# JinPLu/VeloxSeg

Measured on AMD Instinct MI355X. Metric: training patches/s on 128^3 2-mod volumes (fwd+loss+bwd+allreduce+AdamW), higher is better.
Workload: dtype f32

## Files before the change

veloxseg_amd/csrc/pwa_fused.hip:

```cpp
#include "vx_common.h"
#include "../../include/veloxseg_hip.h"

typedef float vx_f32x4 __attribute__((ext_vector_type(4)));
#define VX_MFMA(a, b, c) __builtin_amdgcn_mfma_f32_16x16x4f32((a), (b), (c), 0, 0, 0)

namespace {
template <int T> struct Geo { static constexpr int NT = 16 * T; static constexpr int S = (T == 1) ? 20 : 64; };

template <int T, int NW, bool TR, class Epi>
__device__ __forceinline__ void tile_gemm(int nseg, const float* const (&w)[3], const int (&Kseg)[3], int wsm, int wsk, int Mrows, const float* __restrict__ in, Epi&& epi) {
    constexpr int S = Geo<T>::S;
    const int lane = threadIdx.x & 63, wave = threadIdx.x >> 6, r = lane & 15, q = lane >> 4;
    for (int mt = wave; mt * 16 < Mrows; mt += NW) {
        vx_f32x4 acc[T];
#pragma unroll
        for (int j = 0; j < T; ++j) acc[j] = (vx_f32x4){0.f, 0.f, 0.f, 0.f};
        int kin = 0;
        float a[4][4], an[4][4];
        typedef const __attribute__((address_space(1))) float* gcf;
        typedef const __attribute__((address_space(1))) vx_f32x4* gcf4;
        auto load_a = [&](float (&dst)[4][4], const float* __restrict__ wrow_, int K, int k0) {
            gcf wrow = (gcf)(unsigned long long)wrow_;
#pragma unroll
            for (int c = 0; c < 4; ++c) {
                const int kb = min(k0 + 16 * c, K - 16) + 4 * q;
                if (!TR) {
                    const vx_f32x4 t = *(gcf4)(wrow + kb);
                    dst[c][0] = t[0]; dst[c][1] = t[1]; dst[c][2] = t[2]; dst[c][3] = t[3];
                } else {
#pragma unroll
                    for (int i = 0; i < 4; ++i) dst[c][i] = wrow[(long)(kb + i) * wsk];
                }
            }
// ... 15 lines not shown
                                acc[0] = VX_MFMA(a[c][i], bv.x, acc[0]);
                                acc[1] = VX_MFMA(a[c][i], bv.y, acc[1]);
                                acc[2] = VX_MFMA(a[c][i], bv.z, acc[2]);
                                acc[3] = VX_MFMA(a[c][i], bv.w, acc[3]);
                            } else {
                                acc[0] = VX_MFMA(a[c][i], brow[i * S + r], acc[0]);
                            }
                        }
                    }
                }
                if (k0 + 64 < K) {
#pragma unroll
                    for (int c = 0; c < 4; ++c)
#pragma unroll
                        for (int i = 0; i < 4; ++i) a[c][i] = an[c][i];
                }
            }
            kin += K;
        }
        epi(mt, acc);
    }
}
template <int T, int NW, bool TR, class Epi>
__device__ __forceinline__ void tile_gemm1(const float* w, int K, int wsm, int wsk, int Mrows, const float* __restrict__ in, Epi&& epi) {
    const float* const ws[3] = {w, nullptr, nullptr};
    const int ks[3] = {K, 0, 0};
    tile_gemm<T, NW, TR>(1, ws, ks, wsm, wsk, Mrows, in, epi);
}

template <int T, int NW>
__device__ __forceinline__ void load_tile(float* __restrict__ dst, const float* __restrict__ src , int R, long V, long v0) {
    constexpr int S = Geo<T>::S, RP = 4 * NW, U = 8;
    const int cg = threadIdx.x & 15;
    for (int row0 = threadIdx.x >> 4; row0 < R; row0 += U * RP) {
        if constexpr (T == 4) {
            const long v = v0 + 4 * cg;
            const bool ok = v < V;
            const long vc = ok ? v : 0;
            float4 t[U];
#pragma unroll
            for (int u = 0; u < U; ++u) { const int row = min(row0 + u * RP, R - 1); t[u] = *reinterpret_cast<const float4*>(src + (long)row * V + vc); }
#pragma unroll
            for (int u = 0; u < U; ++u) {
                const int row = row0 + u * RP;
                if (row < R) *reinterpret_cast<float4*>(dst + row * S + 4 * cg) = ok ? t[u] : make_float4(0.f, 0.f, 0.f, 0.f);
            }
        } else {
            const long v = v0 + cg;
            const bool ok = v < V;
            const long vc = ok ? v : 0;
            float t[U];
#pragma unroll
            for (int u = 0; u < U; ++u) { const int row = min(row0 + u * RP, R - 1); t[u] = src[(long)row * V + vc]; }
#pragma unroll
            for (int u = 0; u < U; ++u) {
                const int row = row0 + u * RP;
                if (row < R) dst[row * S + cg] = ok ? t[u] : 0.0f;
            }
        }
    }
}

template <int T, int NW>
__device__ __forceinline__ void tile_ln_stats(const float* __restrict__ X, int C, float eps, float* __restrict__ red, float& mean, float& rstd) {
    constexpr int NT = Geo<T>::NT, S = Geo<T>::S, NP = 64 * NW / NT;
    const int col = threadIdx.x % NT, part = threadIdx.x / NT;
    float s = 0.0f;
    for (int c = part; c < C; c += NP) s += X[c * S + col];
    red[part * NT + col] = s;
    __syncthreads();
    float tot = 0.0f;
#pragma unroll 4
    for (int p_ = 0; p_ < NP; ++p_) tot += red[p_ * NT + col];
    mean = tot / (float)C;
    __syncthreads();
    float qq = 0.0f;
    for (int c = part; c < C; c += NP) { const float d = X[c * S + col] - mean; qq = fmaf(d, d, qq); }
    red[part * NT + col] = qq;
    __syncthreads();
    float var = 0.0f;
#pragma unroll 4
    for (int p_ = 0; p_ < NP; ++p_) var += red[p_ * NT + col];
    rstd = 1.0f / sqrtf(var / (float)C + eps);
}

__device__ __forceinline__ VxDropCtx drop_ctx_dev(const void* seed_ptr, unsigned long long site, float p) {
    VxDrop d;
    d.seed_ptr = p > 0.0f ? (const uint64_t*)seed_ptr : nullptr;
    d.stream = site;
    d.p = p;
    return vx_drop_ctx(d);
}
template <int T>
__device__ __forceinline__ void acc_masks(const VxDropCtx& dc, uint64_t row, long V, long v, float (&m)[4]) {
    if (!dc.on) { m[0] = m[1] = m[2] = m[3] = 1.0f; return; }
    if constexpr (T == 4) vx_masks_vox4(dc, row, V, v, m);
    else { m[0] = vx_drop1(dc, row * (uint64_t)V + (uint64_t)v); m[1] = m[2] = m[3] = 1.0f; }
}
}

struct VxLnPwMod {
    const float *x, *gamma, *beta;
// ... 33 lines not shown
        for (int u = 0; u < U; ++u) {
            const bool in = row0 + u * RP < C;
            const int so = (sub >> 2) * HW2 + ((sub >> 1) & 1) * (2 * gw) + (sub & 1);
            t[u] = xv[(long)c * cstride + so];
            if (in && row0 + (u + 1) * RP < C) {
                c += RP;
                while (c >= C0) { c -= C0; ++sub; }
            }
        }
#pragma unroll
        for (int u = 0; u < U; ++u) {
            const int rw = row0 + u * RP;
            if (rw < C) dst[rw * S + cg] = ok ? t[u] : 0.0f;
        }
    }
}

template <int NW>
__device__ __forceinline__ void stage_vec(float* __restrict__ dst, const float* __restrict__ src, int n, float fill) {
    for (int i = threadIdx.x; i < n; i += 64 * NW) dst[i] = src ? src[i] : fill;
}

template <int T, int NW>
__global__ void __launch_bounds__(64 * NW) vx_ln_pw_fwd_k(VxLnPw p) {
    constexpr int NT = Geo<T>::NT, S = Geo<T>::S, NP = 64 * NW / NT;
    extern __shared__ __attribute__((aligned(16))) float vx_pf_lds[];
    const VxLnPwMod& M = p.m[blockIdx.y];
    const int C = p.C;
    const int Jt = p.J[0] + p.J[1] + p.J[2];
    float* __restrict__ X = vx_pf_lds;
    float* __restrict__ red = X + C * S;
    float* __restrict__ gam = red + NP * NT;
    float* __restrict__ bet = gam + C;
    float* __restrict__ bia = bet + C;
    const int b = blockIdx.x / p.tiles_per_b;
    const long V = p.V, v0 = (long)(blockIdx.x % p.tiles_per_b) * NT;
    stage_vec<NW>(gam, M.gamma, C, 1.0f);
    stage_vec<NW>(bet, M.beta, C, 0.0f);
    {
        int j0 = 0;
        for (int sg = 0; sg < p.NS; ++sg) { stage_vec<NW>(bia + j0, M.b[sg], p.J[sg], 0.0f); j0 += p.J[sg]; }
    }
    if constexpr (T == 1) {
        if (p.s2d) load_tile_s2d<T, NW>(X, M.x + (long)b * C * V, C, p.C0, p.gh, p.gw, V, v0);
        else load_tile<T, NW>(X, M.x + (long)b * C * V, C, V, v0);
    } else load_tile<T, NW>(X, M.x + (long)b * C * V, C, V, v0);
    __syncthreads();
    float mean, rstd;
    tile_ln_stats<T, NW>(X, C, p.eps, red, mean, rstd);
    {
        const int col = threadIdx.x % NT, part = threadIdx.x / NT;
        const bool live = v0 + col < V;
        float* __restrict__ xn = M.xn ? M.xn + (long)b * C * V + v0 + col : nullptr;
        for (int c = part; c < C; c += NP) {
            const float n = fmaf(gam[c], (X[c * S + col] - mean) * rstd, bet[c]);
            X[c * S + col] = n;
            if (xn && live) xn[(long)c * V] = n;
        }
    }
    __syncthreads();
    const int lane = threadIdx.x & 63, r = lane & 15, q = lane >> 4;
    int j0 = 0;
    for (int sg = 0; sg < p.NS; ++sg) {
        const int J = p.J[sg];
        const float* __restrict__ bias = bia + j0;
        float* __restrict__ out = M.out[sg] + (long)b * J * V;
        tile_gemm1<T, NW, false>(M.w[sg], C, C, 1, J, X, [&](int mt, vx_f32x4 (&acc)[T]) {
#pragma unroll
            for (int reg = 0; reg < 4; ++reg) {
                const int m = 16 * mt + 4 * q + reg;
                const float bb = bias[m];
                if constexpr (T == 4) {
                    const long v = v0 + 4 * r;
                    if (v < V) *reinterpret_cast<float4*>(out + (long)m * V + v) = make_float4(acc[0][reg] + bb, acc[1][reg] + bb, acc[2][reg] + bb, acc[3][reg] + bb);
                } else {
                    const long v = v0 + r;
                    if (v < V) out[(long)m * V + v] = acc[0][reg] + bb;
                }
            }
        });
        j0 += J;
    }
}

struct VxLnPwBwdMod {
    const float *x, *gamma;
    const float* w[3];
    const float* dout[3];
    const float* dres;
    float* dx;
    float* part;
};
struct VxLnPwBwd {
    VxLnPwBwdMod m[4];
    int C, NS;
    int J[3];
    long V;
    int tiles_per_b;
    float eps;
    int s2d, C0, gh, gw;
};

template <int T, int NW>
__global__ void __launch_bounds__(64 * NW) vx_ln_pw_bwd_k(VxLnPwBwd p) {
    constexpr int NT = Geo<T>::NT, S = Geo<T>::S, NP = 64 * NW / NT;
    extern __shared__ __attribute__((aligned(16))) float vx_pf_lds[];
    const VxLnPwBwdMod& M = p.m[blockIdx.y];
    const int C = p.C;
    int Jt = 0;
    for (int sg = 0; sg < p.NS; ++sg) Jt += p.J[sg];
    float* __restrict__ D = vx_pf_lds;
    float* __restrict__ X = D + Jt * S;
    float* __restrict__ G = X + C * S;
    float* __restrict__ red = G + C * S;
    float* __restrict__ gam = red + 2 * NP * NT;
    const int b = blockIdx.x / p.tiles_per_b;
    const long V = p.V, v0 = (long)(blockIdx.x % p.tiles_per_b) * NT;
    stage_vec<NW>(gam, M.gamma, C, 1.0f);
    {
        int j0 = 0;
        for (int sg = 0; sg < p.NS; ++sg) {
            load_tile<T, NW>(D + j0 * S, M.dout[sg] + (long)b * p.J[sg] * V, p.J[sg], V, v0);
            j0 += p.J[sg];
        }
    }
    if constexpr (T == 1) {
        if (p.s2d) load_tile_s2d<T, NW>(X, M.x + (long)b * C * V, C, p.C0, p.gh, p.gw, V, v0);
        else load_tile<T, NW>(X, M.x + (long)b * C * V, C, V, v0);
    } else load_tile<T, NW>(X, M.x + (long)b * C * V, C, V, v0);
    __syncthreads();
    const int lane = threadIdx.x & 63, r = lane & 15, q = lane >> 4;
    {
        const float* const ws[3] = {M.w[0], M.w[1], M.w[2]};
        const int ks[3] = {p.J[0], p.J[1], p.J[2]};
        tile_gemm<T, NW, true>(p.NS, ws, ks, 1, C, C, D, [&](int mt, vx_f32x4 (&acc)[T]) {
#pragma unroll
            for (int reg = 0; reg < 4; ++reg) {
                const int m = 16 * mt + 4 * q + reg;
                if constexpr (T == 4) *reinterpret_cast<float4*>(G + m * S + 4 * r) = make_float4(acc[0][reg], acc[1][reg], acc[2][reg], acc[3][reg]);
                else G[m * S + r] = acc[0][reg];
            }
        });
    }
    float mean, rstd;
    tile_ln_stats<T, NW>(X, C, p.eps, red, mean, rstd);
    const bool has_res = M.dres != nullptr && Jt >= C;
    if (has_res) load_tile<T, NW>(D, M.dres + (long)b * C * V, C, V, v0);
    const int col = threadIdx.x % NT, part = threadIdx.x / NT;
    float s1 = 0.0f, s2 = 0.0f;
    for (int c = part; c < C; c += NP) {
        const float xh = (X[c * S + col] - mean) * rstd;
        const float g = G[c * S + col] * gam[c];
        s1 += g;
        s2 = fmaf(g, xh, s2);
    }
    __syncthreads();
    red[part * NT + col] = s1;
    red[(NP + part) * NT + col] = s2;
    __syncthreads();
    float t1 = 0.0f, t2 = 0.0f;
#pragma unroll 4
    for (int p_ = 0; p_ < NP; ++p_) { t1 += red[p_ * NT + col]; t2 += red[(NP + p_) * NT + col]; }
    t1 /= (float)C; t2 /= (float)C;
    const bool live = v0 + col < V;
    float* __restrict__ pp = M.part ? M.part + (long)blockIdx.x * 2 * C : nullptr;
    long s2d_base = 0, HW2 = 0, gd2 = 0;
    if (p.s2d) {
        const long v = live ? v0 + col : 0;
        const int w_ = (int)(v % p.gw), h_ = (int)((v / p.gw) % p.gh), d_ = (int)(v / ((long)p.gw * p.gh));
        HW2 = (long)(2 * p.gh) * (2 * p.gw);
        gd2 = 2 * (V / ((long)p.gh * p.gw));
        s2d_base = (long)b * C * V + (long)(2 * d_) * HW2 + (long)(2 * h_) * (2 * p.gw) + 2 * w_;
    }
    int ssub = p.s2d ? part / p.C0 : 0, sc0 = p.s2d ? part - ssub * p.C0 : 0;
    const long cstr2 = gd2 * HW2;
    for (int c = part; c < C; c += NP) {
        const float xh = (X[c * S + col] - mean) * rstd;
        const float dn = G[c * S + col];
        const float g = dn * gam[c];
        float dg = dn * xh, db = dn;
#pragma unroll
        for (int o = 1; o < NT; o <<= 1) { dg += __shfl_xor(dg, o, 64); db += __shfl_xor(db, o, 64); }
// ... 43 lines not shown
template <int T, int NW>
__global__ void __launch_bounds__(64 * NW) vx_pwa_post_fwd_k(VxPost p) {
    constexpr int NT = Geo<T>::NT, S = Geo<T>::S, NP = 64 * NW / NT;
    extern __shared__ __attribute__((aligned(16))) float vx_pf_lds[];
    const VxPostMod& M = p.m[blockIdx.y];
    const int C = p.C, Cv = p.Cv, R = p.R;
    float* __restrict__ Sx = vx_pf_lds;
    float* __restrict__ Y = Sx + Cv * S;
    float* __restrict__ N = Y + C * S;
    float* __restrict__ Hh = N + C * S;
    float* __restrict__ red = Hh + R * S;
    float* __restrict__ prm = red + NP * NT;
    float* __restrict__ bm = prm, *gam = prm + C, *bet = prm + 2 * C, *b2 = prm + 3 * C, *b1 = prm + 4 * C;
    const int b = blockIdx.x / p.tiles_per_b;
    const long V = p.V, v0 = (long)(blockIdx.x % p.tiles_per_b) * NT;
    const VxDropCtx dm = drop_ctx_dev(p.seed_ptr, M.site_mix, p.p_mix);
    const VxDropCtx d1 = drop_ctx_dev(p.seed_ptr, M.site1, p.p_ffn);
    const VxDropCtx d2 = drop_ctx_dev(p.seed_ptr, M.site2, p.p_ffn);
    stage_vec<NW>(bm, M.bm, C, 0.0f);
    stage_vec<NW>(gam, M.gamma, C, 1.0f);
    stage_vec<NW>(bet, M.beta, C, 0.0f);
    stage_vec<NW>(b2, M.b2, C, 0.0f);
    stage_vec<NW>(b1, M.b1, R, 0.0f);
    load_tile<T, NW>(Sx, M.s + (long)b * Cv * V, Cv, V, v0);
    load_tile<T, NW>(Y, M.x + (long)b * C * V, C, V, v0);
    __syncthreads();
    const int lane = threadIdx.x & 63, r = lane & 15, q = lane >> 4;
    const int cr = T * r;
    const long v = v0 + cr;
    const bool vlive = v < V;
    tile_gemm1<T, NW, false>(M.wm, Cv, Cv, 1, C, Sx, [&](int mt, vx_f32x4 (&acc)[T]) {
#pragma unroll
        for (int reg = 0; reg < 4; ++reg) {
            const int m = 16 * mt + 4 * q + reg;
            const long row = (long)b * C + m;
            float yv[T], mk[4];
            ldv<T>(Y + m * S + cr, yv);
            if (vlive) {
                acc_masks<T>(dm, (uint64_t)row, V, v, mk);
#pragma unroll
                for (int j = 0; j < T; ++j) yv[j] = fmaf(p.alpha, yv[j], (acc[j][reg] + bm[m]) * mk[j]);
                stv<T>(M.y + row * V + v, yv);
            } else {
#pragma unroll
                for (int j = 0; j < T; ++j) yv[j] = 0.0f;
            }
            stv<T>(Y + m * S + cr, yv);
        }
    });
    __syncthreads();
    float mean, rstd;
    tile_ln_stats<T, NW>(Y, C, p.eps, red, mean, rstd);
    {
        const int col = threadIdx.x % NT, part = threadIdx.x / NT;
        for (int c = part; c < C; c += NP) N[c * S + col] = fmaf(gam[c], (Y[c * S + col] - mean) * rstd, bet[c]);
    }
    __syncthreads();
    tile_gemm1<T, NW, false>(M.w1, C, C, 1, R, N, [&](int mt, vx_f32x4 (&acc)[T]) {
#pragma unroll
        for (int reg = 0; reg < 4; ++reg) {
            const int j = 16 * mt + 4 * q + reg;
            float hv[T], mk[4];
            if (vlive) {
                acc_masks<T>(d1, (uint64_t)((long)b * R + j), V, v, mk);
#pragma unroll
                for (int i = 0; i < T; ++i) hv[i] = vx_gelu_fast(acc[i][reg] + b1[j]) * mk[i];
            } else {
#pragma unroll
                for (int i = 0; i < T; ++i) hv[i] = 0.0f;
            }
            stv<T>(Hh + j * S + cr, hv);
        }
    });
    __syncthreads();
    tile_gemm1<T, NW, false>(M.w2, R, R, 1, C, Hh, [&](int mt, vx_f32x4 (&acc)[T]) {
#pragma unroll
        for (int reg = 0; reg < 4; ++reg) {
            const int m = 16 * mt + 4 * q + reg;
            if (vlive) {
                const long row = (long)b * C + m;
                float ov[T], mk[4];
                ldv<T>(Y + m * S + cr, ov);
                acc_masks<T>(d2, (uint64_t)row, V, v, mk);
#pragma unroll
                for (int i = 0; i < T; ++i) ov[i] = fmaf(acc[i][reg] + b2[m], mk[i], ov[i]);
                stv<T>(M.out + row * V + v, ov);
            }
        }
    });
}

template <int T, int NW>
__global__ void __launch_bounds__(64 * NW) vx_pwa_post_bwd_k(VxPost p) {
    constexpr int NT = Geo<T>::NT, S = Geo<T>::S, NP = 64 * NW / NT, NRP = 4 * NW;
    extern __shared__ __attribute__((aligned(16))) float vx_pf_lds[];
    const VxPostMod& M = p.m[blockIdx.y];
    const int C = p.C, Cv = p.Cv, R = p.R;
    float* __restrict__ DO = vx_pf_lds;
// ... 29 lines not shown
#pragma unroll
            for (int j = 0; j < T; ++j) g[j] *= mk[j];
            stv<T>(M.sc_dz + row * V + vq, g);
        } else {
#pragma unroll
            for (int j = 0; j < T; ++j) g[j] = 0.0f;
        }
        stv<T>(DZ + c * S + cq, g);
    }
    float mean, rstd;
    tile_ln_stats<T, NW>(Y, C, p.eps, red, mean, rstd);
    for (int c = part; c < C; c += NP) {
        const float xh = (Y[c * S + col] - mean) * rstd;
        const float n = fmaf(gam[c], xh, bet[c]);
        N[c * S + col] = n;
        Y[c * S + col] = xh;
        if (clive) M.sc_n[((long)b * C + c) * V + v0 + col] = n;
    }
    __syncthreads();
    const int lane = threadIdx.x & 63, r = lane & 15, q = lane >> 4;
    const int cr = T * r;
    const long v = v0 + cr;
    const bool vlive = v < V;
    tile_gemm1<T, NW, false>(M.w1, C, C, 1, R, N, [&](int mt, vx_f32x4 (&acc)[T]) {
#pragma unroll
        for (int reg = 0; reg < 4; ++reg) {
            const int j = 16 * mt + 4 * q + reg;
            float a[T];
#pragma unroll
            for (int i = 0; i < T; ++i) a[i] = acc[i][reg] + b1[j];
            stv<T>(A + j * S + cr, a);
            if (vlive) {
                const long row = (long)b * R + j;
                float mk[4];
                acc_masks<T>(d1, (uint64_t)row, V, v, mk);
#pragma unroll
                for (int i = 0; i < T; ++i) a[i] = vx_gelu_fast(a[i]) * mk[i];
                stv<T>(M.sc_h + row * V + v, a);
            }
        }
    });
    __syncthreads();
    tile_gemm1<T, NW, true>(M.w2, C, 1, R, R, DZ, [&](int mt, vx_f32x4 (&acc)[T]) {
#pragma unroll
        for (int reg = 0; reg < 4; ++reg) {
            const int j = 16 * mt + 4 * q + reg;
            const long row = (long)b * R + j;
            float da[T];
            if (vlive) {
                float mk[4];
                ldv<T>(A + j * S + cr, da);
                acc_masks<T>(d1, (uint64_t)row, V, v, mk);
#pragma unroll
                for (int i = 0; i < T; ++i) da[i] = acc[i][reg] * mk[i] * vx_gelu_grad_fast(da[i]);
                stv<T>(M.sc_da + row * V + v, da);
            } else {
#pragma unroll
                for (int i = 0; i < T; ++i) da[i] = 0.0f;
            }
            stv<T>(A + j * S + cr, da);
        }
    });
    __syncthreads();
    tile_gemm1<T, NW, true>(M.w1, R, 1, C, C, A, [&](int mt, vx_f32x4 (&acc)[T]) {
#pragma unroll
        for (int reg = 0; reg < 4; ++reg) {
            float dn[T];
#pragma unroll
            for (int i = 0; i < T; ++i) dn[i] = acc[i][reg];
            stv<T>(DZ + (16 * mt + 4 * q + reg) * S + cr, dn);
        }
    });
    __syncthreads();
    float s1 = 0.0f, s2 = 0.0f;
    for (int c = part; c < C; c += NP) {
        const float g = DZ[c * S + col] * gam[c];
        s1 += g;
        s2 = fmaf(g, Y[c * S + col], s2);
    }
    red[part * NT + col] = s1;
    red[(NP + part) * NT + col] = s2;
    __syncthreads();
    float t1 = 0.0f, t2 = 0.0f;
#pragma unroll 4
    for (int p_ = 0; p_ < NP; ++p_) { t1 += red[p_ * NT + col]; t2 += red[(NP + p_) * NT + col]; }
    t1 /= (float)C; t2 /= (float)C;
    float rs_[T], t1_[T], t2_[T];
// ... 13 lines not shown
        for (int j = 0; j < T; ++j) { dg = fmaf(dn[j], xh[j], dg); db += dn[j]; }
#pragma unroll
        for (int o = 1; o < 16; o <<= 1) { dg += __shfl_xor(dg, o, 64); db += __shfl_xor(db, o, 64); }
        if (qd == 0) { pp[c] = dg; pp[C + c] = db; }
        if (qlive) {
            float mk[4], dx[T];
            ldv<T>(DO + c * S + cq, dy);
            acc_masks<T>(dm, (uint64_t)row, V, vq, mk);
#pragma unroll
            for (int j = 0; j < T; ++j) {
                dy[j] += rs_[j] * (dn[j] * gam[c] - t1_[j] - xh[j] * t2_[j]);
                dx[j] = p.alpha * dy[j];
                dy[j] *= mk[j];
            }
            stv<T>(M.dxres + row * V + vq, dx);
            stv<T>(M.sc_dmix + row * V + vq, dy);
        } else {
#pragma unroll
            for (int j = 0; j < T; ++j) dy[j] = 0.0f;
        }
        stv<T>(N + c * S + cq, dy);
    }
    __syncthreads();
    tile_gemm1<T, NW, true>(M.wm, C, 1, Cv, Cv, N, [&](int mt, vx_f32x4 (&acc)[T]) {
#pragma unroll
        for (int reg = 0; reg < 4; ++reg) {
            const int m = 16 * mt + 4 * q + reg;
            if (vlive) {
                float o[T];
#pragma unroll
                for (int i = 0; i < T; ++i) o[i] = acc[i][reg];
                stv<T>(M.ds + ((long)b * Cv + m) * V + v, o);
            }
        }
    });
}

static inline int pf_tile_t(long V) { return ((V & 3) == 0 && V >= 2048) ? 4 : 1; }
static inline int pf_nw(long blocks) { return blocks < 256 ? 8 : 4; }

extern "C" int vx_ln_pw_tiles(int B, long V) {
    const int T = pf_tile_t(V);
    return B * vx_cdiv(V, 16 * T);
}

static size_t pf_lds_limit() {
    static size_t lim = 0;
// ... 155 lines not shown
}

struct VxInMlp {
    const float *o, *w1, *b1, *w2, *b2, *dout;
    const double* part;
    float* stats;
    float *out, *dn, *part_dn;
    float *sc_n, *sc_h, *sc_da, *sc_dz;
    int C, R, nparts, tiles_per_b;
    long V;
    float eps, p;
    unsigned long long site;
    const void* seed_ptr;
};
namespace {
template <int NW>
__device__ __forceinline__ void inmlp_stats(const VxInMlp& p, int b, float* __restrict__ mu, float* __restrict__ rs, bool writer) {
    for (int c = threadIdx.x; c < p.C; c += 64 * NW) {
        const long bc = (long)b * p.C + c;
        float mean, rstd;
        if (p.part != nullptr) {
            double s = 0.0, q = 0.0;
            const double* pp = p.part + bc * p.nparts * 2;
            for (int i = 0; i < p.nparts; ++i) { s += pp[2 * i]; q += pp[2 * i + 1]; }
            const double m = s / (double)p.V;
            double var = q / (double)p.V - m * m;
            var = var < 0.0 ? 0.0 : var;
            mean = (float)m;
            rstd = (float)(1.0 / sqrt(var + (double)p.eps));
            if (writer) { p.stats[2 * bc] = mean; p.stats[2 * bc + 1] = rstd; }
        } else {
            mean = p.stats[2 * bc];
            rstd = p.stats[2 * bc + 1];
        }
        mu[c] = mean;
        rs[c] = rstd;
    }
}
}

template <int NW>
__global__ void __launch_bounds__(64 * NW) vx_inmlp_fwd_k(VxInMlp p) {
    constexpr int T = 1, NT = 16, S = Geo<1>::S, NP = 64 * NW / NT;
    extern __shared__ __attribute__((aligned(16))) float vx_pf_lds[];
    const int C = p.C, R = p.R;
    float* __restrict__ O = vx_pf_lds;
    float* __restrict__ N = O + C * S;
    float* __restrict__ Hh = N + C * S;
    float* __restrict__ mu = Hh + R * S, *rs = mu + C, *b2 = rs + C, *b1 = b2 + C;
    const int b = blockIdx.x / p.tiles_per_b, tile = blockIdx.x % p.tiles_per_b;
    const long V = p.V, v0 = (long)tile * NT;
    const VxDropCtx d2 = drop_ctx_dev(p.seed_ptr, p.site, p.p);
    inmlp_stats<NW>(p, b, mu, rs, tile == 0);
    stage_vec<NW>(b2, p.b2, C, 0.0f);
    stage_vec<NW>(b1, p.b1, R, 0.0f);
    load_tile<T, NW>(O, p.o + (long)b * C * V, C, V, v0);
    __syncthreads();
    {
        const int col = threadIdx.x % NT, part = threadIdx.x / NT;
        for (int c = part; c < C; c += NP) N[c * S + col] = (O[c * S + col] - mu[c]) * rs[c];
    }
    __syncthreads();
    const int lane = threadIdx.x & 63, r = lane & 15, q = lane >> 4;
    const long v = v0 + r;
    const bool vlive = v < V;
    tile_gemm1<T, NW, false>(p.w1, C, C, 1, R, N, [&](int mt, vx_f32x4 (&acc)[T]) {
#pragma unroll
        for (int reg = 0; reg < 4; ++reg) {
            const int j = 16 * mt + 4 * q + reg;
            Hh[j * S + r] = vlive ? vx_gelu_fast(acc[0][reg] + b1[j]) : 0.0f;
        }
    });
    __syncthreads();
    tile_gemm1<T, NW, false>(p.w2, R, R, 1, C, Hh, [&](int mt, vx_f32x4 (&acc)[T]) {
#pragma unroll
        for (int reg = 0; reg < 4; ++reg) {
            const int m = 16 * mt + 4 * q + reg;
            if (vlive) {
                const long idx = ((long)b * C + m) * V + v;
                p.out[idx] = fmaf(acc[0][reg] + b2[m], vx_drop1(d2, (uint64_t)idx), O[m * S + r]);
            }
        }
    });
}

template <int NW>
__global__ void __launch_bounds__(64 * NW) vx_inmlp_bwd_k(VxInMlp p) {
    constexpr int T = 1, NT = 16, S = Geo<1>::S, NP = 64 * NW / NT;
    extern __shared__ __attribute__((aligned(16))) float vx_pf_lds[];
    const int C = p.C, R = p.R;
    float* __restrict__ DZ = vx_pf_lds;
    float* __restrict__ N = DZ + C * S;
    float* __restrict__ A = N + C * S;
    float* __restrict__ mu = A + R * S, *rs = mu + C, *b1 = rs + C;
    const int b = blockIdx.x / p.tiles_per_b, tile = blockIdx.x % p.tiles_per_b;
    const long V = p.V, v0 = (long)tile * NT;
    const VxDropCtx d2 = drop_ctx_dev(p.seed_ptr, p.site, p.p);
    const int col = threadIdx.x % NT, part = threadIdx.x / NT;
    const bool clive = v0 + col < V;
    inmlp_stats<NW>(p, b, mu, rs, false);
    stage_vec<NW>(b1, p.b1, R, 0.0f);
    load_tile<T, NW>(N, p.o + (long)b * C * V, C, V, v0);
    load_tile<T, NW>(DZ, p.dout + (long)b * C * V, C, V, v0);
    __syncthreads();
    for (int c = part; c < C; c += NP) {
        const long idx = ((long)b * C + c) * V + v0 + col;
        const float g = clive ? DZ[c * S + col] * vx_drop1(d2, (uint64_t)idx) : 0.0f;
        const float nh = clive ? (N[c * S + col] - mu[c]) * rs[c] : 0.0f;
        DZ[c * S + col] = g;
        N[c * S + col] = nh;
        if (clive) { p.sc_dz[idx] = g; p.sc_n[idx] = nh; }
    }
    __syncthreads();
    const int lane = threadIdx.x & 63, r = lane & 15, q = lane >> 4;
    const long v = v0 + r;
    const bool vlive = v < V;
    tile_gemm1<T, NW, false>(p.w1, C, C, 1, R, N, [&](int mt, vx_f32x4 (&acc)[T]) {
#pragma unroll
        for (int reg = 0; reg < 4; ++reg) {
            const int j = 16 * mt + 4 * q + reg;
            const float a = acc[0][reg] + b1[j];
            A[j * S + r] = a;
            if (vlive) p.sc_h[((long)b * R + j) * V + v] = vx_gelu_fast(a);
        }
    });
    __syncthreads();
    tile_gemm1<T, NW, true>(p.w2, C, 1, R, R, DZ, [&](int mt, vx_f32x4 (&acc)[T]) {
#pragma unroll
        for (int reg = 0; reg < 4; ++reg) {
            const int j = 16 * mt + 4 * q + reg;
            const float da = vlive ? acc[0][reg] * vx_gelu_grad_fast(A[j * S + r]) : 0.0f;
            A[j * S + r] = da;
            if (vlive) p.sc_da[((long)b * R + j) * V + v] = da;
        }
    });
    __syncthreads();
    tile_gemm1<T, NW, true>(p.w1, R, 1, C, C, A, [&](int mt, vx_f32x4 (&acc)[T]) {
#pragma unroll
        for (int reg = 0; reg < 4; ++reg) {
            const int m = 16 * mt + 4 * q + reg;
            const float dn = vlive ? acc[0][reg] : 0.0f;
            if (vlive) p.dn[((long)b * C + m) * V + v] = dn;
            float s1 = dn, s2 = dn * N[m * S + r];
#pragma unroll
            for (int o_ = 1; o_ < 16; o_ <<= 1) { s1 += __shfl_xor(s1, o_, 64); s2 += __shfl_xor(s2, o_, 64); }
            if (r == 0) {
                float* __restrict__ pp = p.part_dn + (((long)b * C + m) * p.tiles_per_b + tile) * 2;
                pp[0] = s1; pp[1] = s2;
            }
        }
    });
}

extern "C" int vx_inmlp_ok(int C, int R, long V) {
    if (C % 16 || R % 16 || C < 16 || R < 16 || C > 256 || V < 1) return 0;
    const size_t lds = ((size_t)(2 * C + R) * 20 + 3 * C + R) * sizeof(float);
    return lds <= pf_lds_budget() ? 1 : 0;
}
extern "C" int vx_inmlp_tiles(long V) { return vx_cdiv(V, 16); }

// ... 34 lines not shown
```

Baseline: 1118.

## Pipeline weight-fragment prefetch across GEMM tiles and overlap with tile loads in fused kernels

Restructures the fused pointwise GEMM helper into a software-pipelined loop that prefetches the next weight fragment across m-tiles and segments, and issues the first fragment before staging and LDS loads so global latency overlaps other work. The forward LN+pointwise kernel merges its per-segment GEMMs into one flat m-tile loop, and the backward kernel splits n-columns across waves when there are few m-tiles. It also adds LDS-only fence barriers, occupancy hints in launch bounds, early residual fetches held in registers, and an unrolled partial-sum reduction. The cost is higher register pressure and more complex control flow.

```diff
diff --git a/veloxseg_amd/csrc/pwa_fused.hip b/veloxseg_amd/csrc/pwa_fused.hip
--- a/veloxseg_amd/csrc/pwa_fused.hip
+++ b/veloxseg_amd/csrc/pwa_fused.hip
@@ -7,8 +7,112 @@
 namespace {
 template <int T> struct Geo { static constexpr int NT = 16 * T; static constexpr int S = (T == 1) ? 20 : 64; };
 
+typedef const __attribute__((address_space(1))) float* gcf;
+typedef const __attribute__((address_space(1))) vx_f32x4* gcf4;
+struct AFrag { float a[4][4]; };
+
+__device__ __forceinline__ void vx_bar() {
+    __builtin_amdgcn_fence(__ATOMIC_RELEASE, "workgroup", "local");
+    __builtin_amdgcn_s_barrier();
+    __builtin_amdgcn_fence(__ATOMIC_ACQUIRE, "workgroup", "local");
+}
+
+template <bool TR, int KP>
+__device__ __forceinline__ void load_a(float (&dst)[4][4], const float* __restrict__ wrow_, int K, int k0, int wsk) {
+    const int q = (threadIdx.x & 63) >> 4;
+    gcf wrow = (gcf)(unsigned long long)wrow_;
+#pragma unroll
+    for (int c = 0; c < KP; ++c) {
+        const int kb = min(k0 + 16 * c, K - 16) + 4 * q;
+        if (!TR) {
+            const vx_f32x4 t = *(gcf4)(wrow + kb);
+            dst[c][0] = t[0]; dst[c][1] = t[1]; dst[c][2] = t[2]; dst[c][3] = t[3];
+        } else {
+#pragma unroll
+            for (int i = 0; i < 4; ++i) dst[c][i] = wrow[(long)(kb + i) * wsk];
+        }
+    }
+}
+template <bool TR, int KP, class WRow>
+__device__ __forceinline__ void tile_gemm_first(AFrag& f, int wl, int K0, int wsk, int Mrows, WRow&& wrow) {
+    if (wl * 16 < Mrows) load_a<TR, KP>(f.a, wrow(wl, 0), K0, 0, wsk);
+}
+
+template <int T, int NJ, bool TR, int KP, class WRow, class Epi>
+__device__ __forceinline__ void tile_gemm(AFrag& pre, int wl, int WG, int j0, int nseg, int K0, int K1, int K2, int wsk, int Mrows, WRow&& wrow, const float* __restrict__ in,
+                                          Epi&& epi) {
+    constexpr int S = Geo<T>::S, KC = 16 * KP;
+    static_assert(NJ == T || (T == 4 && (NJ == 1 || NJ == 2)), "n-tile sharing: T = 4 only");
+    const int lane = threadIdx.x & 63, r = lane & 15, q = lane >> 4;
+    if (wl * 16 >= Mrows) return;
+    float (&a)[4][4] = pre.a;
+    auto Kof = [&](int s) { return s == 0 ? K0 : (s == 1 ? K1 : K2); };
+    float an[4][4];
+    vx_f32x4 acc[NJ];
+    auto chunk = [&](int K, int k0, int kin) {
+        if (kin == 0 && k0 == 0) {
+#pragma unroll
+            for (int j = 0; j < NJ; ++j) acc[j] = (vx_f32x4){0.f, 0.f, 0.f, 0.f};
+        }
+#pragma unroll
+        for (int c = 0; c < KP; ++c) {
+            if (k0 + 16 * c < K) {
+                const float* __restrict__ brow = in + (long)(kin + k0 + 16 * c + 4 * q) * S;
+#pragma unroll
+                for (int i = 0; i < 4; ++i) {
+                    if constexpr (T == 4 && NJ == 4) {
+                        const float4 bv = *reinterpret_cast<const float4*>(brow + i * S + 4 * r);
+                        acc[0] = VX_MFMA(a[c][i], bv.x, acc[0]);
+                        acc[1] = VX_MFMA(a[c][i], bv.y, acc[1]);
+                        acc[2] = VX_MFMA(a[c][i], bv.z, acc[2]);
+                        acc[3] = VX_MFMA(a[c][i], bv.w, acc[3]);
+                    } else if constexpr (T == 4 && NJ == 2) {
+                        const float2 bv = *reinterpret_cast<const float2*>(brow + i * S + 4 * r + j0);
+                        acc[0] = VX_MFMA(a[c][i], bv.x, acc[0]);
+                        acc[1] = VX_MFMA(a[c][i], bv.y, acc[1]);
+                    } else if constexpr (T == 4) {
+                        acc[0] = VX_MFMA(a[c][i], brow[i * S + 4 * r + j0], acc[0]);
+                    } else {
+                        acc[0] = VX_MFMA(a[c][i], brow[i * S + r], acc[0]);
+                    }
+                }
+            }
+        }
+    };
+    int mt = wl, sg = 0, k0 = 0, kin = 0;
+    for (;;) {
+        const int K = Kof(sg);
+        int nmt = mt, nsg = sg, nk0 = k0 + KC;
+        if (nk0 >= K) { nk0 = 0; if (++nsg >= nseg) { nsg = 0; nmt += WG; } }
+        if (nmt * 16 >= Mrows) break;
+        load_a<TR, KP>(an, wrow(nmt, nsg), Kof(nsg), nk0, wsk);
+        chunk(K, k0, kin);
+        if (nk0 == 0) {
+            kin += K;
+            if (nsg == 0) { epi(mt, acc); kin = 0; }
+        }
+#pragma unroll
+        for (int c = 0; c < KP; ++c)
+#pragma unroll
+            for (int i = 0; i < 4; ++i) a[c][i] = an[c][i];
+        mt = nmt; sg = nsg; k0 = nk0;
+    }
+    chunk(Kof(sg), k0, kin);
+    epi(mt, acc);
+}
 template <int T, int NW, bool TR, class Epi>
-__device__ __forceinline__ void tile_gemm(int nseg, const float* const (&w)[3], const int (&Kseg)[3], int wsm, int wsk, int Mrows, const float* __restrict__ in, Epi&& epi) {
+__device__ __forceinline__ void tile_gemm1(AFrag& pre, const float* w, int K, int wsm, int wsk, int Mrows, const float* __restrict__ in, Epi&& epi) {
+    const int r = threadIdx.x & 15;
+    tile_gemm<T, T, TR, 4>(pre, threadIdx.x >> 6, NW, 0, 1, K, 0, 0, wsk, Mrows, [&](int mt, int) { return w + (long)(16 * mt + r) * wsm; }, in, epi);
+}
+template <int NW, bool TR>
+__device__ __forceinline__ void tile_gemm1_first(AFrag& f, const float* w, int K, int wsm, int wsk, int Mrows) {
+    const int r = threadIdx.x & 15;
+    tile_gemm_first<TR, 4>(f, threadIdx.x >> 6, K, wsk, Mrows, [&](int mt, int) { return w + (long)(16 * mt + r) * wsm; });
+}
+
+template <int T, int NW, bool TR, class Epi>
+__device__ __forceinline__ void tile_gemm_seq(int nseg, const float* const (&w)[3], const int (&Kseg)[3], int wsm, int wsk, int Mrows, const float* __restrict__ in, Epi&& epi) {
     constexpr int S = Geo<T>::S;
     const int lane = threadIdx.x & 63, wave = threadIdx.x >> 6, r = lane & 15, q = lane >> 4;
     for (int mt = wave; mt * 16 < Mrows; mt += NW) {
@@ -70,42 +174,47 @@
     }
 }
 template <int T, int NW, bool TR, class Epi>
-__device__ __forceinline__ void tile_gemm1(const float* w, int K, int wsm, int wsk, int Mrows, const float* __restrict__ in, Epi&& epi) {
+__device__ __forceinline__ void tile_gemm1_seq(const float* w, int K, int wsm, int wsk, int Mrows, const float* __restrict__ in, Epi&& epi) {
     const float* const ws[3] = {w, nullptr, nullptr};
     const int ks[3] = {K, 0, 0};
-    tile_gemm<T, NW, TR>(1, ws, ks, wsm, wsk, Mrows, in, epi);
-}
-
+    tile_gemm_seq<T, NW, TR>(1, ws, ks, wsm, wsk, Mrows, in, epi);
+}
+
+template <int T> struct TileVec { typedef float type; };
+template <> struct TileVec<4> { typedef float4 type; };
+template <int T, int NW, int U>
+__device__ __forceinline__ void tile_fetch(typename TileVec<T>::type (&t)[U], const float* __restrict__ src, int R, long V, long v0, int row0) {
+    constexpr int RP = 4 * NW;
+    const int cg = threadIdx.x & 15;
+    const long v = v0 + T * cg;
+    const long vc = v < V ? v : 0;
+#pragma unroll
+    for (int u = 0; u < U; ++u) {
+        const int row = row0 + u * RP;
+        if (row < R) t[u] = *reinterpret_cast<const typename TileVec<T>::type*>(src + (long)row * V + vc);
+    }
+}
+template <int T, int NW, int U>
+__device__ __forceinline__ void tile_commit(float* __restrict__ dst, const typename TileVec<T>::type (&t)[U], int R, long V, long v0, int row0) {
+    constexpr int S = Geo<T>::S, RP = 4 * NW;
+    const int cg = threadIdx.x & 15;
+    const bool ok = v0 + T * cg < V;
+#pragma unroll
+    for (int u = 0; u < U; ++u) {
+        const int row = row0 + u * RP;
+        if (row < R) {
+            if constexpr (T == 4) *reinterpret_cast<float4*>(dst + row * S + 4 * cg) = ok ? t[u] : make_float4(0.f, 0.f, 0.f, 0.f);
+            else dst[row * S + cg] = ok ? t[u] : 0.0f;
+        }
+    }
+}
 template <int T, int NW>
-__device__ __forceinline__ void load_tile(float* __restrict__ dst, const float* __restrict__ src , int R, long V, long v0) {
-    constexpr int S = Geo<T>::S, RP = 4 * NW, U = 8;
-    const int cg = threadIdx.x & 15;
-    for (int row0 = threadIdx.x >> 4; row0 < R; row0 += U * RP) {
-        if constexpr (T == 4) {
-            const long v = v0 + 4 * cg;
-            const bool ok = v < V;
-            const long vc = ok ? v : 0;
-            float4 t[U];
-#pragma unroll
-            for (int u = 0; u < U; ++u) { const int row = min(row0 + u * RP, R - 1); t[u] = *reinterpret_cast<const float4*>(src + (long)row * V + vc); }
-#pragma unroll
-            for (int u = 0; u < U; ++u) {
-                const int row = row0 + u * RP;
-                if (row < R) *reinterpret_cast<float4*>(dst + row * S + 4 * cg) = ok ? t[u] : make_float4(0.f, 0.f, 0.f, 0.f);
-            }
-        } else {
-            const long v = v0 + cg;
-            const bool ok = v < V;
-            const long vc = ok ? v : 0;
-            float t[U];
-#pragma unroll
-            for (int u = 0; u < U; ++u) { const int row = min(row0 + u * RP, R - 1); t[u] = src[(long)row * V + vc]; }
-#pragma unroll
-            for (int u = 0; u < U; ++u) {
-                const int row = row0 + u * RP;
-                if (row < R) dst[row * S + cg] = ok ? t[u] : 0.0f;
-            }
-        }
+__device__ __forceinline__ void load_tile(float* __restrict__ dst, const float* __restrict__ src , int R, long V, long v0, int batch0 = 0) {
+    constexpr int RP = 4 * NW, U = T == 4 ? 4 : 8;
+    for (int row0 = (threadIdx.x >> 4) + batch0 * U * RP; row0 < R; row0 += U * RP) {
+        typename TileVec<T>::type t[U];
+        tile_fetch<T, NW, U>(t, src, R, V, v0, row0);
+        tile_commit<T, NW, U>(dst, t, R, V, v0, row0);
     }
 }
 
@@ -116,16 +225,16 @@
     float s = 0.0f;
     for (int c = part; c < C; c += NP) s += X[c * S + col];
     red[part * NT + col] = s;
-    __syncthreads();
+    vx_bar();
     float tot = 0.0f;
 #pragma unroll 4
     for (int p_ = 0; p_ < NP; ++p_) tot += red[p_ * NT + col];
     mean = tot / (float)C;
-    __syncthreads();
+    vx_bar();
     float qq = 0.0f;
     for (int c = part; c < C; c += NP) { const float d = X[c * S + col] - mean; qq = fmaf(d, d, qq); }
     red[part * NT + col] = qq;
-    __syncthreads();
+    vx_bar();
     float var = 0.0f;
 #pragma unroll 4
     for (int p_ = 0; p_ < NP; ++p_) var += red[p_ * NT + col];
@@ -205,7 +314,7 @@
 }
 
 template <int T, int NW>
-__global__ void __launch_bounds__(64 * NW) vx_ln_pw_fwd_k(VxLnPw p) {
+__global__ void __launch_bounds__(64 * NW, (T == 4 ? 6 : 1)) vx_ln_pw_fwd_k(VxLnPw p) {
     constexpr int NT = Geo<T>::NT, S = Geo<T>::S, NP = 64 * NW / NT;
     extern __shared__ __attribute__((aligned(16))) float vx_pf_lds[];
     const VxLnPwMod& M = p.m[blockIdx.y];
@@ -218,6 +327,17 @@
     float* __restrict__ bia = bet + C;
     const int b = blockIdx.x / p.tiles_per_b;
     const long V = p.V, v0 = (long)(blockIdx.x % p.tiles_per_b) * NT;
+    const int lane = threadIdx.x & 63, r = lane & 15, q = lane >> 4;
+    const int J0 = p.J[0], J01 = J0 + p.J[1];
+    const float* const w0 = M.w[0], *const w1 = M.w[1], *const w2 = M.w[2];
+    auto wrow = [&](int mt, int) {
+        const int m0 = 16 * mt;
+        return m0 < J0 ? w0 + (long)(m0 + r) * C : (m0 < J01 ? w1 + (long)(m0 - J0 + r) * C : w2 + (long)(m0 - J01 + r) * C);
+    };
+    AFrag fa;
+    const bool k16 = T == 4 && C == 16;
+    if constexpr (T == 4) { if (k16) tile_gemm_first<false, 1>(fa, threadIdx.x >> 6, C, 1, Jt, wrow); }
+    if (!k16) tile_gemm_first<false, 4>(fa, threadIdx.x >> 6, C, 1, Jt, wrow);
     stage_vec<NW>(gam, M.gamma, C, 1.0f);
     stage_vec<NW>(bet, M.beta, C, 0.0f);
     {
@@ -228,7 +348,7 @@
         if (p.s2d) load_tile_s2d<T, NW>(X, M.x + (long)b * C * V, C, p.C0, p.gh, p.gw, V, v0);
         else load_tile<T, NW>(X, M.x + (long)b * C * V, C, V, v0);
     } else load_tile<T, NW>(X, M.x + (long)b * C * V, C, V, v0);
-    __syncthreads();
+    vx_bar();
     float mean, rstd;
     tile_ln_stats<T, NW>(X, C, p.eps, red, mean, rstd);
     {
@@ -241,29 +361,26 @@
             if (xn && live) xn[(long)c * V] = n;
         }
     }
-    __syncthreads();
-    const int lane = threadIdx.x & 63, r = lane & 15, q = lane >> 4;
-    int j0 = 0;
-    for (int sg = 0; sg < p.NS; ++sg) {
-        const int J = p.J[sg];
-        const float* __restrict__ bias = bia + j0;
-        float* __restrict__ out = M.out[sg] + (long)b * J * V;
-        tile_gemm1<T, NW, false>(M.w[sg], C, C, 1, J, X, [&](int mt, vx_f32x4 (&acc)[T]) {
-#pragma unroll
-            for (int reg = 0; reg < 4; ++reg) {
-                const int m = 16 * mt + 4 * q + reg;
-                const float bb = bias[m];
-                if constexpr (T == 4) {
-                    const long v = v0 + 4 * r;
-                    if (v < V) *reinterpret_cast<float4*>(out + (long)m * V + v) = make_float4(acc[0][reg] + bb, acc[1][reg] + bb, acc[2][reg] + bb, acc[3][reg] + bb);
-                } else {
-                    const long v = v0 + r;
-                    if (v < V) out[(long)m * V + v] = acc[0][reg] + bb;
-                }
-            }
-        });
-        j0 += J;
-    }
+    vx_bar();
+    auto epi = [&](int mt, vx_f32x4 (&acc)[T]) {
+        const int m0 = 16 * mt;
+        const int sg = m0 < J0 ? 0 : (m0 < J01 ? 1 : 2), joff = sg == 0 ? 0 : (sg == 1 ? J0 : J01), J = sg == 0 ? J0 + 0 : (sg == 1 ? J01 - J0 : Jt - J01);
+        float* __restrict__ out = (sg == 0 ? M.out[0] : (sg == 1 ? M.out[1] : M.out[2])) + (long)b * J * V;
+#pragma unroll
+        for (int reg = 0; reg < 4; ++reg) {
+            const int m = m0 - joff + 4 * q + reg;
+            const float bb = bia[joff + m];
+            if constexpr (T == 4) {
+                const long v = v0 + 4 * r;
+                if (v < V) *reinterpret_cast<float4*>(out + (long)m * V + v) = make_float4(acc[0][reg] + bb, acc[1][reg] + bb, acc[2][reg] + bb, acc[3][reg] + bb);
+            } else {
+                const long v = v0 + r;
+                if (v < V) out[(long)m * V + v] = acc[0][reg] + bb;
+            }
+        }
+    };
+    if constexpr (T == 4) { if (k16) tile_gemm<T, T, false, 1>(fa, threadIdx.x >> 6, NW, 0, 1, C, 0, 0, 1, Jt, wrow, X, epi); }
+    if (!k16) tile_gemm<T, T, false, 4>(fa, threadIdx.x >> 6, NW, 0, 1, C, 0, 0, 1, Jt, wrow, X, epi);
 }
 
 struct VxLnPwBwdMod {
@@ -285,7 +402,7 @@
 };
 
 template <int T, int NW>
-__global__ void __launch_bounds__(64 * NW) vx_ln_pw_bwd_k(VxLnPwBwd p) {
+__global__ void __launch_bounds__(64 * NW, (T == 4 ? 5 : 1)) vx_ln_pw_bwd_k(VxLnPwBwd p) {
     constexpr int NT = Geo<T>::NT, S = Geo<T>::S, NP = 64 * NW / NT;
     extern __shared__ __attribute__((aligned(16))) float vx_pf_lds[];
     const VxLnPwBwdMod& M = p.m[blockIdx.y];
@@ -299,6 +416,22 @@
     float* __restrict__ gam = red + 2 * NP * NT;
     const int b = blockIdx.x / p.tiles_per_b;
     const long V = p.V, v0 = (long)(blockIdx.x % p.tiles_per_b) * NT;
+    const int lane = threadIdx.x & 63, wave = threadIdx.x >> 6, r = lane & 15, q = lane >> 4;
+    const int tiles = C >> 4;
+    const int nsp = (T == 4 && 4 * tiles <= NW) ? 4 : ((T == 4 && 2 * tiles <= NW) ? 2 : 1);
+    const int WG = NW / nsp, wl = wave % WG;
+    const float* const w0 = M.w[0], *const w1 = M.w[1], *const w2 = M.w[2];
+    auto wrow = [&](int mt, int sg) { return (sg == 0 ? w0 : (sg == 1 ? w1 : w2)) + 16 * mt + r; };
+    AFrag fa;
+    if constexpr (T == 4) {
+        if (nsp == 4) tile_gemm_first<true, 1>(fa, wl, p.J[0], C, C, wrow);
+        else tile_gemm_first<true, 4>(fa, wl, p.J[0], C, C, wrow);
+    }
+    constexpr int RU = 4, RP = 4 * NW;
+    const bool has_res = M.dres != nullptr && Jt >= C;
+    const bool res_early = T == 4 && has_res && C <= RU * RP;
+    typename TileVec<T>::type tres[RU];
+    if (res_early) tile_fetch<T, NW, RU>(tres, M.dres + (long)b * C * V, C, V, v0, threadIdx.x >> 4);
     stage_vec<NW>(gam, M.gamma, C, 1.0f);
     {
         int j0 = 0;
@@ -311,24 +444,37 @@
         if (p.s2d) load_tile_s2d<T, NW>(X, M.x + (long)b * C * V, C, p.C0, p.gh, p.gw, V, v0);
         else load_tile<T, NW>(X, M.x + (long)b * C * V, C, V, v0);
     } else load_tile<T, NW>(X, M.x + (long)b * C * V, C, V, v0);
-    __syncthreads();
-    const int lane = threadIdx.x & 63, r = lane & 15, q = lane >> 4;
-    {
+    vx_bar();
+    if constexpr (T == 4) {
+        if (nsp == 4) {
+            tile_gemm<T, 1, true, 1>(fa, wl, WG, wave / WG, p.NS, p.J[0], p.J[1], p.J[2], C, C, wrow, D, [&](int mt, vx_f32x4 (&acc)[1]) {
+#pragma unroll
+                for (int reg = 0; reg < 4; ++reg) G[(16 * mt + 4 * q + reg) * S + 4 * r + wave / WG] = acc[0][reg];
+            });
+        } else if (nsp == 2) {
+            tile_gemm<T, 2, true, 4>(fa, wl, WG, 2 * (wave / WG), p.NS, p.J[0], p.J[1], p.J[2], C, C, wrow, D, [&](int mt, vx_f32x4 (&acc)[2]) {
+#pragma unroll
+                for (int reg = 0; reg < 4; ++reg) *reinterpret_cast<float2*>(G + (16 * mt + 4 * q + reg) * S + 4 * r + 2 * (wave / WG)) = make_float2(acc[0][reg], acc[1][reg]);
+            });
+        }
+        if (nsp == 1) {
+            tile_gemm<T, T, true, 4>(fa, wl, WG, 0, p.NS, p.J[0], p.J[1], p.J[2], C, C, wrow, D, [&](int mt, vx_f32x4 (&acc)[T]) {
+#pragma unroll
+                for (int reg = 0; reg < 4; ++reg) *reinterpret_cast<float4*>(G + (16 * mt + 4 * q + reg) * S + 4 * r) = make_float4(acc[0][reg], acc[1][reg], acc[2][reg], acc[3][reg]);
+            });
+        }
+    } else {
         const float* const ws[3] = {M.w[0], M.w[1], M.w[2]};
         const int ks[3] = {p.J[0], p.J[1], p.J[2]};
-        tile_gemm<T, NW, true>(p.NS, ws, ks, 1, C, C, D, [&](int mt, vx_f32x4 (&acc)[T]) {
-#pragma unroll
-            for (int reg = 0; reg < 4; ++reg) {
-                const int m = 16 * mt + 4 * q + reg;
-                if constexpr (T == 4) *reinterpret_cast<float4*>(G + m * S + 4 * r) = make_float4(acc[0][reg], acc[1][reg], acc[2][reg], acc[3][reg]);
-                else G[m * S + r] = acc[0][reg];
-            }
+        tile_gemm_seq<T, NW, true>(p.NS, ws, ks, 1, C, C, D, [&](int mt, vx_f32x4 (&acc)[T]) {
+#pragma unroll
+            for (int reg = 0; reg < 4; ++reg) G[(16 * mt + 4 * q + reg) * S + r] = acc[0][reg];
         });
     }
     float mean, rstd;
     tile_ln_stats<T, NW>(X, C, p.eps, red, mean, rstd);
-    const bool has_res = M.dres != nullptr && Jt >= C;
-    if (has_res) load_tile<T, NW>(D, M.dres + (long)b * C * V, C, V, v0);
+    if (res_early) tile_commit<T, NW, RU>(D, tres, C, V, v0, threadIdx.x >> 4);
+    else if (has_res) load_tile<T, NW>(D, M.dres + (long)b * C * V, C, V, v0);
     const int col = threadIdx.x % NT, part = threadIdx.x / NT;
     float s1 = 0.0f, s2 = 0.0f;
     for (int c = part; c < C; c += NP) {
@@ -337,10 +483,10 @@
         s1 += g;
         s2 = fmaf(g, xh, s2);
     }
-    __syncthreads();
+    vx_bar();
     red[part * NT + col] = s1;
     red[(NP + part) * NT + col] = s2;
-    __syncthreads();
+    vx_bar();
     float t1 = 0.0f, t2 = 0.0f;
 #pragma unroll 4
     for (int p_ = 0; p_ < NP; ++p_) { t1 += red[p_ * NT + col]; t2 += red[(NP + p_) * NT + col]; }
@@ -430,14 +576,16 @@
     stage_vec<NW>(bet, M.beta, C, 0.0f);
     stage_vec<NW>(b2, M.b2, C, 0.0f);
     stage_vec<NW>(b1, M.b1, R, 0.0f);
+    AFrag fa;
+    tile_gemm1_first<NW, false>(fa, M.wm, Cv, Cv, 1, C);
     load_tile<T, NW>(Sx, M.s + (long)b * Cv * V, Cv, V, v0);
     load_tile<T, NW>(Y, M.x + (long)b * C * V, C, V, v0);
-    __syncthreads();
+    vx_bar();
     const int lane = threadIdx.x & 63, r = lane & 15, q = lane >> 4;
     const int cr = T * r;
     const long v = v0 + cr;
     const bool vlive = v < V;
-    tile_gemm1<T, NW, false>(M.wm, Cv, Cv, 1, C, Sx, [&](int mt, vx_f32x4 (&acc)[T]) {
+    tile_gemm1<T, NW, false>(fa, M.wm, Cv, Cv, 1, C, Sx, [&](int mt, vx_f32x4 (&acc)[T]) {
 #pragma unroll
         for (int reg = 0; reg < 4; ++reg) {
             const int m = 16 * mt + 4 * q + reg;
@@ -456,15 +604,16 @@
             stv<T>(Y + m * S + cr, yv);
         }
     });
-    __syncthreads();
+    tile_gemm1_first<NW, false>(fa, M.w1, C, C, 1, R);
+    vx_bar();
     float mean, rstd;
     tile_ln_stats<T, NW>(Y, C, p.eps, red, mean, rstd);
     {
         const int col = threadIdx.x % NT, part = threadIdx.x / NT;
         for (int c = part; c < C; c += NP) N[c * S + col] = fmaf(gam[c], (Y[c * S + col] - mean) * rstd, bet[c]);
     }
-    __syncthreads();
-    tile_gemm1<T, NW, false>(M.w1, C, C, 1, R, N, [&](int mt, vx_f32x4 (&acc)[T]) {
+    vx_bar();
+    tile_gemm1<T, NW, false>(fa, M.w1, C, C, 1, R, N, [&](int mt, vx_f32x4 (&acc)[T]) {
 #pragma unroll
         for (int reg = 0; reg < 4; ++reg) {
             const int j = 16 * mt + 4 * q + reg;
@@ -480,8 +629,9 @@
             stv<T>(Hh + j * S + cr, hv);
         }
     });
-    __syncthreads();
-    tile_gemm1<T, NW, false>(M.w2, R, R, 1, C, Hh, [&](int mt, vx_f32x4 (&acc)[T]) {
+    tile_gemm1_first<NW, false>(fa, M.w2, R, R, 1, C);
+    vx_bar();
+    tile_gemm1<T, NW, false>(fa, M.w2, R, R, 1, C, Hh, [&](int mt, vx_f32x4 (&acc)[T]) {
 #pragma unroll
         for (int reg = 0; reg < 4; ++reg) {
             const int m = 16 * mt + 4 * q + reg;
@@ -557,7 +707,7 @@
     const int cr = T * r;
     const long v = v0 + cr;
     const bool vlive = v < V;
-    tile_gemm1<T, NW, false>(M.w1, C, C, 1, R, N, [&](int mt, vx_f32x4 (&acc)[T]) {
+    tile_gemm1_seq<T, NW, false>(M.w1, C, C, 1, R, N, [&](int mt, vx_f32x4 (&acc)[T]) {
 #pragma unroll
         for (int reg = 0; reg < 4; ++reg) {
             const int j = 16 * mt + 4 * q + reg;
@@ -576,7 +726,7 @@
         }
     });
     __syncthreads();
-    tile_gemm1<T, NW, true>(M.w2, C, 1, R, R, DZ, [&](int mt, vx_f32x4 (&acc)[T]) {
+    tile_gemm1_seq<T, NW, true>(M.w2, C, 1, R, R, DZ, [&](int mt, vx_f32x4 (&acc)[T]) {
 #pragma unroll
         for (int reg = 0; reg < 4; ++reg) {
             const int j = 16 * mt + 4 * q + reg;
@@ -597,7 +747,7 @@
         }
     });
     __syncthreads();
-    tile_gemm1<T, NW, true>(M.w1, R, 1, C, C, A, [&](int mt, vx_f32x4 (&acc)[T]) {
+    tile_gemm1_seq<T, NW, true>(M.w1, R, 1, C, C, A, [&](int mt, vx_f32x4 (&acc)[T]) {
 #pragma unroll
         for (int reg = 0; reg < 4; ++reg) {
             float dn[T];
@@ -657,7 +807,7 @@
         stv<T>(N + c * S + cq, dy);
     }
     __syncthreads();
-    tile_gemm1<T, NW, true>(M.wm, C, 1, Cv, Cv, N, [&](int mt, vx_f32x4 (&acc)[T]) {
+    tile_gemm1_seq<T, NW, true>(M.wm, C, 1, Cv, Cv, N, [&](int mt, vx_f32x4 (&acc)[T]) {
 #pragma unroll
         for (int reg = 0; reg < 4; ++reg) {
             const int m = 16 * mt + 4 * q + reg;
@@ -859,7 +1009,13 @@
         if (p.part != nullptr) {
             double s = 0.0, q = 0.0;
             const double* pp = p.part + bc * p.nparts * 2;
-            for (int i = 0; i < p.nparts; ++i) { s += pp[2 * i]; q += pp[2 * i + 1]; }
+            for (int i0 = 0; i0 < p.nparts; i0 += 8) {
+                double ls[8], lq[8];
+#pragma unroll
+                for (int u = 0; u < 8; ++u) { const int i = min(i0 + u, p.nparts - 1); ls[u] = pp[2 * i]; lq[u] = pp[2 * i + 1]; }
+#pragma unroll
+                for (int u = 0; u < 8; ++u) if (i0 + u < p.nparts) { s += ls[u]; q += lq[u]; }
+            }
             const double m = s / (double)p.V;
             double var = q / (double)p.V - m * m;
             var = var < 0.0 ? 0.0 : var;
@@ -888,28 +1044,34 @@
     const int b = blockIdx.x / p.tiles_per_b, tile = blockIdx.x % p.tiles_per_b;
     const long V = p.V, v0 = (long)tile * NT;
     const VxDropCtx d2 = drop_ctx_dev(p.seed_ptr, p.site, p.p);
+    AFrag fa;
+    tile_gemm1_first<NW, false>(fa, p.w1, C, C, 1, R);
+    float t0[8];
+    tile_fetch<T, NW, 8>(t0, p.o + (long)b * C * V, C, V, v0, threadIdx.x >> 4);
     inmlp_stats<NW>(p, b, mu, rs, tile == 0);
     stage_vec<NW>(b2, p.b2, C, 0.0f);
     stage_vec<NW>(b1, p.b1, R, 0.0f);
-    load_tile<T, NW>(O, p.o + (long)b * C * V, C, V, v0);
-    __syncthreads();
+    tile_commit<T, NW, 8>(O, t0, C, V, v0, threadIdx.x >> 4);
+    load_tile<T, NW>(O, p.o + (long)b * C * V, C, V, v0, 1);
+    vx_bar();
     {
         const int col = threadIdx.x % NT, part = threadIdx.x / NT;
         for (int c = part; c < C; c += NP) N[c * S + col] = (O[c * S + col] - mu[c]) * rs[c];
     }
-    __syncthreads();
+    vx_bar();
     const int lane = threadIdx.x & 63, r = lane & 15, q = lane >> 4;
     const long v = v0 + r;
     const bool vlive = v < V;
-    tile_gemm1<T, NW, false>(p.w1, C, C, 1, R, N, [&](int mt, vx_f32x4 (&acc)[T]) {
+    tile_gemm1<T, NW, false>(fa, p.w1, C, C, 1, R, N, [&](int mt, vx_f32x4 (&acc)[T]) {
 #pragma unroll
         for (int reg = 0; reg < 4; ++reg) {
             const int j = 16 * mt + 4 * q + reg;
             Hh[j * S + r] = vlive ? vx_gelu_fast(acc[0][reg] + b1[j]) : 0.0f;
         }
     });
-    __syncthreads();
-    tile_gemm1<T, NW, false>(p.w2, R, R, 1, C, Hh, [&](int mt, vx_f32x4 (&acc)[T]) {
+    tile_gemm1_first<NW, false>(fa, p.w2, R, R, 1, C);
+    vx_bar();
+    tile_gemm1<T, NW, false>(fa, p.w2, R, R, 1, C, Hh, [&](int mt, vx_f32x4 (&acc)[T]) {
 #pragma unroll
         for (int reg = 0; reg < 4; ++reg) {
             const int m = 16 * mt + 4 * q + reg;
@@ -952,7 +1114,7 @@
     const int lane = threadIdx.x & 63, r = lane & 15, q = lane >> 4;
     const long v = v0 + r;
     const bool vlive = v < V;
-    tile_gemm1<T, NW, false>(p.w1, C, C, 1, R, N, [&](int mt, vx_f32x4 (&acc)[T]) {
+    tile_gemm1_seq<T, NW, false>(p.w1, C, C, 1, R, N, [&](int mt, vx_f32x4 (&acc)[T]) {
 #pragma unroll
         for (int reg = 0; reg < 4; ++reg) {
             const int j = 16 * mt + 4 * q + reg;
@@ -962,7 +1124,7 @@
         }
     });
     __syncthreads();
-    tile_gemm1<T, NW, true>(p.w2, C, 1, R, R, DZ, [&](int mt, vx_f32x4 (&acc)[T]) {
+    tile_gemm1_seq<T, NW, true>(p.w2, C, 1, R, R, DZ, [&](int mt, vx_f32x4 (&acc)[T]) {
 #pragma unroll
         for (int reg = 0; reg < 4; ++reg) {
             const int j = 16 * mt + 4 * q + reg;
@@ -972,7 +1134,7 @@
         }
     });
     __syncthreads();
-    tile_gemm1<T, NW, true>(p.w1, R, 1, C, C, A, [&](int mt, vx_f32x4 (&acc)[T]) {
+    tile_gemm1_seq<T, NW, true>(p.w1, R, 1, C, C, A, [&](int mt, vx_f32x4 (&acc)[T]) {
 #pragma unroll
         for (int reg = 0; reg < 4; ++reg) {
             const int m = 16 * mt + 4 * q + reg;
```

Result: faster. 1132 (median of 6 runs) (+1.3%).
